# serenedb/serenedb

Measured on NVIDIA H100. Metric: filter->GROUP BY throughput (BASELINE.json configs[1]; bm25 object = configs[2]), higher is better.
Workload: dtype int64+f64

## Files before the change

### serenedb_b200/csrc/column_kernels.cuh

```cuda
#pragma once

#include "device_common.cuh"

namespace sdbg {

constexpr int kMaxPreds = 4;

struct ColDev {
  const void* values;
  const uint64_t* validity;
  int32_t type;
  int32_t pad;
};
struct PredDev {
  ColDev col;
  int32_t op;
  int32_t pad;
  int64_t lo_i, hi_i;
  double lo_f, hi_f;
};
struct PredSet {
  PredDev p[kMaxPreds];
  int32_t n;
  int32_t pad;
};

__device__ __forceinline__ bool col_valid(const ColDev& c, uint64_t r) {
  return c.validity == nullptr || ((__ldg(c.validity + (r >> 6)) >> (r & 63)) & 1ull);
}
__device__ __forceinline__ bool cmp_i64(int op, long long v, long long lo, long long hi) {
  switch (op) {
    case 0: return v < lo; case 1: return v <= lo; case 2: return v > lo; case 3: return v >= lo;
    case 4: return v == lo; case 5: return v != lo; default: return v >= lo && v <= hi;
  }
}
__device__ __forceinline__ bool cmp_f64(int op, double v, double lo, double hi) {
  switch (op) {
    case 0: return v < lo; case 1: return v <= lo; case 2: return v > lo; case 3: return v >= lo;
    case 4: return v == lo; case 5: return v != lo; default: return v >= lo && v <= hi;
  }
}

__device__ __forceinline__ uint32_t pred2(const PredDev& p, uint64_t r, uint64_t rows) {
  uint32_t valid = 3u;
  if (p.col.validity) valid = (col_valid(p.col, r) ? 1u : 0u) | ((r + 1 < rows && col_valid(p.col, r + 1)) ? 2u : 0u);
  if (p.op == 7) return (~valid) & 3u;
  if (p.op == 8) return valid;
  uint32_t m = 0;
  if (p.col.type == 2) {
    const int2 v = *reinterpret_cast<const int2*>(static_cast<const int*>(p.col.values) + r);
    m = (cmp_i64(p.op, v.x, p.lo_i, p.hi_i) ? 1u : 0u) | (cmp_i64(p.op, v.y, p.lo_i, p.hi_i) ? 2u : 0u);
  } else {
    const uint4 raw = ld_stream_v4(static_cast<const char*>(p.col.values) + r * 8);
    if (p.col.type == 1) {
      const double a = __longlong_as_double((static_cast<long long>(raw.y) << 32) | raw.x);
      const double b = __longlong_as_double((static_cast<long long>(raw.w) << 32) | raw.z);
      m = (cmp_f64(p.op, a, p.lo_f, p.hi_f) ? 1u : 0u) | (cmp_f64(p.op, b, p.lo_f, p.hi_f) ? 2u : 0u);
    } else {
      const long long a = (static_cast<long long>(raw.y) << 32) | raw.x;
      const long long b = (static_cast<long long>(raw.w) << 32) | raw.z;
      m = (cmp_i64(p.op, a, p.lo_i, p.hi_i) ? 1u : 0u) | (cmp_i64(p.op, b, p.lo_i, p.hi_i) ? 2u : 0u);
    }
  }
  return m & valid;
}

__device__ __forceinline__ uint32_t preds2(const PredSet& ps, uint64_t r, uint64_t rows) {
  uint32_t m = (r + 1 < rows) ? 3u : 1u;
#pragma unroll
  for (int i = 0; i < kMaxPreds; ++i) {
    if (i < ps.n) m &= pred2(ps.p[i], r, rows);
  }
  return m;
}

__device__ __forceinline__ bool pred1(const PredDev& p, uint64_t r) {
  const bool valid = col_valid(p.col, r);
  if (p.op >= 7) return (p.op == 8) == valid;
  if (!valid) return false;
  bool in;
  if (p.col.type == 1) {
    const double v = __ldg(static_cast<const double*>(p.col.values) + r);
    in = v >= p.lo_f && v <= p.hi_f;
  } else {
    const long long v = p.col.type == 2 ? static_cast<long long>(__ldg(static_cast<const int*>(p.col.values) + r))
                                        : __ldg(static_cast<const long long*>(p.col.values) + r);
    in = v >= p.lo_i && v <= p.hi_i;
  }
  return in != (p.op == 5);
}

__device__ __forceinline__ bool preds_row(const PredSet& ps, uint64_t r) {
  if (ps.n == 0) return true;
  if (!pred1(ps.p[0], r)) return false;
#pragma unroll 1
  for (int i = 1; i < ps.n; ++i)
    if (!pred1(ps.p[i], r)) return false;
  return true;
}

__device__ __forceinline__ void load2_i64(const ColDev& c, uint64_t r, long long& a, long long& b) {
  if (c.type == 2) {
    const int2 v = *reinterpret_cast<const int2*>(static_cast<const int*>(c.values) + r);
    a = v.x; b = v.y;
  } else {
    const uint4 raw = ld_stream_v4(static_cast<const char*>(c.values) + r * 8);
    a = (static_cast<long long>(raw.y) << 32) | raw.x;
    b = (static_cast<long long>(raw.w) << 32) | raw.z;
  }
}
__device__ __forceinline__ void load2_f64(const ColDev& c, uint64_t r, double& a, double& b) {
  const uint4 raw = ld_stream_v4(static_cast<const char*>(c.values) + r * 8);
  a = __longlong_as_double((static_cast<long long>(raw.y) << 32) | raw.x);
  b = __longlong_as_double((static_cast<long long>(raw.w) << 32) | raw.z);
}

__global__ void __launch_bounds__(256)
filter_bitmap_kernel(const PredSet ps, uint64_t rows, unsigned long long* __restrict__ mask_out) {
  const uint64_t words = (rows + 63) / 64;
  const uint32_t lane = threadIdx.x & 31u;
  for (uint64_t w = (uint64_t(blockIdx.x) * blockDim.x + threadIdx.x) >> 5; w < words;
       w += (uint64_t(gridDim.x) * blockDim.x) >> 5) {
    const uint64_t r = w * 64 + 2ull * lane;
    const uint32_t m = r < rows ? preds2(ps, r, rows) : 0u;
    const uint32_t b0 = __ballot_sync(kFull, m & 1u);
    const uint32_t b1 = __ballot_sync(kFull, m & 2u);
    if (lane == 0) {
      unsigned long long x = 0;
      for (int l = 0; l < 32; ++l) {
        x |= static_cast<unsigned long long>((b0 >> l) & 1u) << (2 * l);
        x |= static_cast<unsigned long long>((b1 >> l) & 1u) << (2 * l + 1);
      }
      mask_out[w] = x;
    }
  }
}

struct CountSumOut {
  unsigned long long count;
  unsigned long long sum_lo;
  long long sum_hi;
  double sum_f;
};

__device__ __forceinline__ void add128(unsigned long long& lo, long long& hi, long long v) {
  const unsigned long long nlo = lo + static_cast<unsigned long long>(v);
  hi += (v < 0 ? -1ll : 0ll) + (nlo < lo ? 1ll : 0ll);
  lo = nlo;
}
__device__ __forceinline__ void add128u(unsigned long long& lo, long long& hi, unsigned long long alo, long long ahi) {
  const unsigned long long nlo = lo + alo;
  hi += ahi + (nlo < lo ? 1ll : 0ll);
  lo = nlo;
}

__global__ void __launch_bounds__(256)
filter_count_sum_kernel(const PredSet ps, const ColDev sum_col, int has_sum, uint64_t rows,
                        CountSumOut* __restrict__ partials, unsigned int* __restrict__ done_counter, CountSumOut* host_out,
                        unsigned long long* host_seq, unsigned long long seq) {
  unsigned long long cnt = 0, lo = 0;
  long long hi = 0;
  double sf = 0.0;
  const uint64_t stride = uint64_t(gridDim.x) * blockDim.x * 2ull;
  for (uint64_t r = (uint64_t(blockIdx.x) * blockDim.x + threadIdx.x) * 2ull; r < rows; r += stride) {
    const uint32_t m = preds2(ps, r, rows);
    if (has_sum) {
      uint32_t mv = m;
      if (sum_col.validity) mv &= (col_valid(sum_col, r) ? 1u : 0u) | ((r + 1 < rows && col_valid(sum_col, r + 1)) ? 2u : 0u);
      if (sum_col.type == 1) {
        double a, b; load2_f64(sum_col, r, a, b);
        if (mv & 1u) sf += a;
        if (mv & 2u) sf += b;
      } else {
        long long a, b; load2_i64(sum_col, r, a, b);
        if (mv & 1u) add128(lo, hi, a);
        if (mv & 2u) add128(lo, hi, b);
      }
    }
    cnt += __popc(m);
  }
#pragma unroll
  for (int o = 16; o > 0; o >>= 1) {
    cnt += __shfl_xor_sync(kFull, cnt, o);
    const unsigned long long olo = __shfl_xor_sync(kFull, lo, o);
    const long long ohi = __shfl_xor_sync(kFull, hi, o);
    add128u(lo, hi, olo, ohi);
    sf += __shfl_xor_sync(kFull, sf, o);
  }
  __shared__ CountSumOut s[8];
  __shared__ bool s_last;
  const uint32_t lane = threadIdx.x & 31u, warp = threadIdx.x >> 5;
  if (lane == 0) { s[warp].count = cnt; s[warp].sum_lo = lo; s[warp].sum_hi = hi; s[warp].sum_f = sf; }
  __syncthreads();
  if (threadIdx.x == 0) {
    CountSumOut t = s[0];
    for (uint32_t w = 1; w < blockDim.x / 32u; ++w) {
      t.count += s[w].count; add128u(t.sum_lo, t.sum_hi, s[w].sum_lo, s[w].sum_hi); t.sum_f += s[w].sum_f;
    }
    partials[blockIdx.x] = t;
    __threadfence();
    s_last = atomicAdd(done_counter, 1u) == gridDim.x - 1u;
  }
  __syncthreads();
  if (s_last) {
    __threadfence();
    CountSumOut t = {0, 0, 0, 0.0};
    for (uint32_t b = threadIdx.x; b < gridDim.x; b += blockDim.x) {
      const volatile CountSumOut* p = partials + b;
      t.count += p->count; add128u(t.sum_lo, t.sum_hi, p->sum_lo, p->sum_hi); t.sum_f += p->sum_f;
    }
#pragma unroll
    for (int o = 16; o > 0; o >>= 1) {
      t.count += __shfl_xor_sync(kFull, t.count, o);
      const unsigned long long olo = __shfl_xor_sync(kFull, t.sum_lo, o);
      const long long ohi = __shfl_xor_sync(kFull, t.sum_hi, o);
      add128u(t.sum_lo, t.sum_hi, olo, ohi);
      t.sum_f += __shfl_xor_sync(kFull, t.sum_f, o);
    }
    __syncthreads();
    if (lane == 0) s[warp] = t;
    __syncthreads();
    if (threadIdx.x == 0) {
      CountSumOut r = s[0];
      for (uint32_t w = 1; w < blockDim.x / 32u; ++w) {
        r.count += s[w].count; add128u(r.sum_lo, r.sum_hi, s[w].sum_lo, s[w].sum_hi); r.sum_f += s[w].sum_f;
      }
      partials[gridDim.x] = r;
      if (host_out != nullptr) {
        *host_out = r;
        __threadfence_system();
        if (host_seq != nullptr) *reinterpret_cast<volatile unsigned long long*>(host_seq) = seq;
      }
      *done_counter = 0u;
    }
  }
}

struct GroupSlot {
  unsigned long long count;
  long long sum_lo;
  long long sum_hi;
  double sum_f;
};
static_assert(sizeof(GroupSlot) == 32, "one L2 sector per group");

struct GroupByParams {
  PredSet ps;
  ColDev key, sum_i, sum_f;
  int32_t has_sum_i, has_sum_f;
  int32_t wide_int;
  int32_t count_f;
  int64_t key_min;
  uint64_t key_span;
  uint64_t rows;
  GroupSlot* table;
  unsigned long long* cnt_f;
  unsigned long long* out_of_range;
};

__device__ __forceinline__ void group_update(const GroupByParams& P, long long key, long long v, bool v_ok,
                                             double w, bool w_ok) {
  const unsigned long long idx = static_cast<unsigned long long>(key - P.key_min);
  if (idx >= P.key_span) { atomicAdd(P.out_of_range, 1ull); return; }
  GroupSlot* g = P.table + idx;
  atomicAdd(&g->count, 1ull);
  if (P.has_sum_i && v_ok) {
    if (P.wide_int) {
      atomicAdd(reinterpret_cast<unsigned long long*>(&g->sum_lo), static_cast<unsigned long long>(v) & 0xFFFFFFFFull);
      atomicAdd(reinterpret_cast<unsigned long long*>(&g->sum_hi), static_cast<unsigned long long>(v >> 32));
    } else {
      atomicAdd(reinterpret_cast<unsigned long long*>(&g->sum_lo), static_cast<unsigned long long>(v));
    }
  }
  if (P.has_sum_f && w_ok) {
    atomicAdd(&g->sum_f, w);
    if (P.count_f) atomicAdd(P.cnt_f + idx, 1ull);
  }
}

template <int kUnroll>
__global__ void __launch_bounds__(256)
filter_groupby_kernel(const GroupByParams P) {
  const uint64_t tile = uint64_t(blockDim.x) * 2ull * kUnroll;
  for (uint64_t base = uint64_t(blockIdx.x) * tile; base < P.rows; base += uint64_t(gridDim.x) * tile) {
    uint32_t m[kUnroll];
    long long k0[kUnroll], k1[kUnroll], v0[kUnroll], v1[kUnroll];
    double w0[kUnroll], w1[kUnroll];
#pragma unroll
    for (int u = 0; u < kUnroll; ++u) {
      const uint64_t r = base + (uint64_t(u) * blockDim.x + threadIdx.x) * 2ull;
      m[u] = 0; k0[u] = k1[u] = v0[u] = v1[u] = 0; w0[u] = w1[u] = 0.0;
      if (r < P.rows) {
        m[u] = preds2(P.ps, r, P.rows);
        load2_i64(P.key, r, k0[u], k1[u]);
        if (P.has_sum_i) load2_i64(P.sum_i, r, v0[u], v1[u]);
        if (P.has_sum_f) load2_f64(P.sum_f, r, w0[u], w1[u]);
      }
    }
#pragma unroll
    for (int u = 0; u < kUnroll; ++u) {
      if (!m[u]) continue;
      const uint64_t r = base + (uint64_t(u) * blockDim.x + threadIdx.x) * 2ull;
      bool vi0 = true, vi1 = true, wf0 = true, wf1 = true;
      if (P.has_sum_i && P.sum_i.validity) { vi0 = col_valid(P.sum_i, r); vi1 = r + 1 < P.rows && col_valid(P.sum_i, r + 1); }
      if (P.has_sum_f && P.sum_f.validity) { wf0 = col_valid(P.sum_f, r); wf1 = r + 1 < P.rows && col_valid(P.sum_f, r + 1); }
      if (m[u] & 1u) group_update(P, k0[u], v0[u], vi0, w0[u], wf0);
      if (m[u] & 2u) group_update(P, k1[u], v1[u], vi1, w1[u], wf1);
    }
  }
}

constexpr int kMaxStreams = 7;

struct ForBlockDev { long long base; uint32_t bits; uint32_t off8; };
constexpr uint32_t kForGroupRows = 2048;
constexpr int kTypeFor = 3;

struct TmaGroupByParams {
  const void* src[kMaxStreams];
  int32_t elem[kMaxStreams];
  uint32_t off[kMaxStreams + 1];
  int32_t n_streams;
  int32_t n_preds;
  uint32_t pred_off[kMaxPreds];
  int32_t pred_type[kMaxPreds];
  int32_t pred_negate[kMaxPreds];
  int64_t pred_lo[kMaxPreds];
  uint64_t pred_span[kMaxPreds];
  uint32_t key_off, sum_i_off, sum_f_off;
  int32_t key_type, sum_i_type;
  int32_t has_sum_i, has_sum_f;
  int32_t wide_int;
  int32_t debug_skip;
  int32_t pack_shift, pack_tables;
  int64_t pack_bias;
  int64_t key_min;
  uint64_t key_span;
  uint64_t rows;
  GroupSlot* table;
  unsigned long long* out_of_range;
  const uint8_t* skip;
  const ForBlockDev* hdr[kMaxStreams];
  int32_t pred_stream[kMaxPreds];
  int32_t key_stream, sum_i_stream;
};
constexpr uint32_t kZoneRows = 2048;

__host__ __device__ __forceinline__ long long fkey(long long bits) { return bits ^ ((bits >> 63) & 0x7FFFFFFFFFFFFFFFll); }

__device__ __forceinline__ void fix_limbs(double w, int limb, int eunit, long long& l0, long long& l1) {
  const long long bits = __double_as_longlong(w);
  const int ex = int((bits >> 52) & 0x7FF);
  unsigned long long mant = static_cast<unsigned long long>(bits) & 0xFFFFFFFFFFFFFull;
  if (ex) mant |= 1ull << 52;
  const int s = (ex ? ex : 1) - 1075 - eunit;
  unsigned long long lo, hi = 0ull;
  if (s >= 0) { lo = mant << s; if (s) hi = mant >> (64 - s); }
  else lo = s > -64 ? mant >> (-s) : 0ull;
  l0 = static_cast<long long>(lo & ((1ull << limb) - 1ull));
  l1 = static_cast<long long>((lo >> limb) | (hi << (64 - limb)));
  if (bits < 0) { l0 = -l0; l1 = -l1; }
}
__host__ __device__ __forceinline__ double fix_total(long long s0, long long s1, int limb, int eunit) {
  long long hi = s1 >> (64 - limb);
  unsigned long long lo = static_cast<unsigned long long>(s1) << limb;
  const unsigned long long lo2 = lo + static_cast<unsigned long long>(s0);
  hi += (s0 >> 63) + (lo2 < lo ? 1 : 0);
  lo = lo2;
  const bool neg = hi < 0;
  if (neg) { lo = ~lo + 1ull; hi = ~hi + (lo == 0ull ? 1 : 0); }
  const double mag = static_cast<double>(static_cast<unsigned long long>(hi)) * 18446744073709551616.0 + static_cast<double>(lo);
  return scalbn(neg ? -mag : mag, eunit);
}

template <int kType>
__device__ __forceinline__ void load2(const unsigned char* col, uint32_t r, long long (&v)[2]) {
  if (kType == 2) {
    const int2 x = *reinterpret_cast<const int2*>(col + size_t(r) * 4u);
    v[0] = x.x; v[1] = x.y;
  } else {
    const longlong2 x = *reinterpret_cast<const longlong2*>(col + size_t(r) * 8u);
    v[0] = x.x; v[1] = x.y;
  }
}
template <int kType>
__device__ __forceinline__ uint32_t range2(const unsigned char* col, uint32_t r, long long lo, unsigned long long span) {
  long long v[2];
  load2<kType>(col, r, v);
  if (kType == 1) { v[0] = fkey(v[0]); v[1] = fkey(v[1]); }
  return (static_cast<unsigned long long>(v[0] - lo) <= span ? 1u : 0u) | (static_cast<unsigned long long>(v[1] - lo) <= span ? 2u : 0u);
}
__device__ __forceinline__ void unpack2(const unsigned char* col, uint32_t r, const uint4 h, long long (&v)[2]) {
  const unsigned long long* w = reinterpret_cast<const unsigned long long*>(col);
  const uint32_t bits = h.z;
  const long long base = static_cast<long long>((static_cast<unsigned long long>(h.y) << 32) | h.x);
  const unsigned long long mask = bits >= 64u ? ~0ull : (1ull << bits) - 1ull;
#pragma unroll
  for (int j = 0; j < 2; ++j) {
    const uint32_t bit = (r + uint32_t(j)) * bits, wi = bit >> 6, sh = bit & 63u;
    unsigned long long x = w[wi] >> sh;
    if (sh + bits > 64u) x |= w[wi + 1] << (64u - sh);
    v[j] = base + static_cast<long long>(x & mask);
  }
}
__device__ __forceinline__ uint32_t range2_for(const unsigned char* col, uint32_t r, const uint4 h, long long lo, unsigned long long span) {
  long long v[2];
  unpack2(col, r, h, v);
  return (static_cast<unsigned long long>(v[0] - lo) <= span ? 1u : 0u) | (static_cast<unsigned long long>(v[1] - lo) <= span ? 2u : 0u);
}

constexpr int kGroupByStages = 3;
constexpr int kGroupByTileRows = 512;
constexpr int kGroupByConsumerWarps = 8;
template <bool kPacked, bool kFor>
__global__ void __launch_bounds__((kGroupByConsumerWarps + 1) * 32)
filter_groupby_tma_kernel(const TmaGroupByParams P) {
  constexpr int kStages = kGroupByStages, kTileRows = kGroupByTileRows, kConsumerWarps = kGroupByConsumerWarps;
  extern __shared__ __align__(128) unsigned char smem[];
  __shared__ __align__(8) uint64_t full_bar[kStages], empty_bar[kStages];
  static_assert(!kFor || (kForGroupRows % kTileRows == 0 && kTileRows % 128 == 0), "a tile's packed slice must be 16-byte aligned");

  const uint32_t tid = threadIdx.x, warp = tid >> 5, lane = tid & 31u;
  if (tid == 0) {
    for (int s = 0; s < kStages; ++s) { mbar_init(&full_bar[s], 1u); mbar_init(&empty_bar[s], kConsumerWarps); }
    asm volatile("fence.mbarrier_init.release.cluster;" ::: "memory");
  }
  __syncthreads();
  const uint32_t stage_bytes = P.off[P.n_streams];
  const uint64_t n_tiles = (P.rows + kTileRows - 1) / kTileRows;
  uint4* const pk_hdr = reinterpret_cast<uint4*>(smem + size_t(kStages) * stage_bytes);

  if (warp == kConsumerWarps) {
    if (kFor) {
      const bool mine = lane < uint32_t(P.n_streams);
      const ForBlockDev* hp = mine ? P.hdr[lane] : nullptr;
      const char* src = mine ? static_cast<const char*>(P.src[lane]) : nullptr;
      const uint32_t elem = mine ? uint32_t(P.elem[lane]) : 0u, soff = mine ? P.off[lane] : 0u;
      auto header = [&](uint64_t t) { return __ldg(reinterpret_cast<const uint4*>(hp + (t * kTileRows) / kForGroupRows)); };
      uint4 nh = make_uint4(0u, 0u, 0u, 0u);
      uint64_t nh_tile = ~0ull;
      uint32_t it = 0;
      for (uint64_t tile = blockIdx.x; tile < n_tiles; tile += gridDim.x) {
        if (P.skip != nullptr && P.skip[(tile * kTileRows) / kZoneRows]) continue;
        uint4 h = make_uint4(0u, 0u, 0u, 0u);
        if (hp != nullptr) h = nh_tile == tile ? nh : header(tile);
        const uint64_t next = tile + gridDim.x;
        if (hp != nullptr && next < n_tiles && (P.skip == nullptr || !P.skip[(next * kTileRows) / kZoneRows])) { nh = header(next); nh_tile = next; }
        const uint32_t st = it % kStages, use = it / kStages;
        ++it;
        const uint64_t row0 = tile * kTileRows;
        const uint32_t nrows = uint32_t(min(static_cast<unsigned long long>(kTileRows), static_cast<unsigned long long>(P.rows - row0)));
        uint32_t bytes = 0u;
        const char* g = nullptr;
        if (hp != nullptr) {
          bytes = (nrows * h.z + 127u) / 128u * 16u;
          g = src + uint64_t(h.w) * 8u + (row0 % kForGroupRows) * h.z / 8u;
        } else if (mine) {
          bytes = (nrows * elem + 15u) & ~15u;
          g = src + row0 * elem;
        }
        const uint32_t total = __reduce_add_sync(kFull, bytes);
        if (lane == 0) mbar_wait(&empty_bar[st], (use & 1u) ^ 1u);
        for (int s = 0; s < P.n_streams; ++s) {
          uint4 x;
          x.x = __shfl_sync(kFull, h.x, s); x.y = __shfl_sync(kFull, h.y, s); x.z = __shfl_sync(kFull, h.z, s); x.w = __shfl_sync(kFull, h.w, s);
          if (lane == 0) pk_hdr[st * kMaxStreams + s] = x;
        }
        if (lane == 0) mbar_arrive_expect_tx(&full_bar[st], total);
        __syncwarp();
        if (bytes != 0u) bulk_g2s(smem + size_t(st) * stage_bytes + soff, g, bytes, &full_bar[st]);
      }
      return;
    }
    if (lane == 0) {
      uint32_t it = 0;
      for (uint64_t tile = blockIdx.x; tile < n_tiles; tile += gridDim.x) {
        if (P.skip != nullptr && P.skip[(tile * kTileRows) / kZoneRows]) continue;
        const uint32_t st = it % kStages, use = it / kStages;
        ++it;
        mbar_wait(&empty_bar[st], (use & 1u) ^ 1u);
        const uint64_t row0 = tile * kTileRows;
        const uint32_t nrows = uint32_t(min(static_cast<unsigned long long>(kTileRows), static_cast<unsigned long long>(P.rows - row0)));
        uint32_t total = 0;
        for (int s = 0; s < P.n_streams; ++s) total += (nrows * uint32_t(P.elem[s]) + 15u) & ~15u;
        mbar_arrive_expect_tx(&full_bar[st], total);
        unsigned char* dst = smem + size_t(st) * stage_bytes;
        for (int s = 0; s < P.n_streams; ++s) {
          const uint32_t bytes = (nrows * uint32_t(P.elem[s]) + 15u) & ~15u;
          bulk_g2s(dst + P.off[s], static_cast<const char*>(P.src[s]) + row0 * uint64_t(P.elem[s]), bytes, &full_bar[st]);
        }
      }
    }
    return;
  }

  uint32_t it = 0;
  for (uint64_t tile = blockIdx.x; tile < n_tiles; tile += gridDim.x) {
    if (P.skip != nullptr && P.skip[(tile * kTileRows) / kZoneRows]) continue;
    const uint32_t st = it % kStages, use = it / kStages;
    ++it;
    mbar_wait(&full_bar[st], use & 1u);
    const unsigned char* base = smem + size_t(st) * stage_bytes;
    const uint64_t row0 = tile * kTileRows;
    const uint32_t nrows = uint32_t(min(static_cast<unsigned long long>(kTileRows), static_cast<unsigned long long>(P.rows - row0)));
    const uint32_t pack_word = kPacked ? uint32_t(tile % uint64_t(P.pack_tables)) : 0u;
    const uint4* const hst = pk_hdr + st * kMaxStreams;
    for (uint32_t rb = warp * 64u; rb < nrows; rb += kConsumerWarps * 64u) {
      const uint32_t r = rb + 2u * lane;
      uint32_t m = r + 1u < nrows ? 3u : r < nrows ? 1u : 0u;
#pragma unroll
      for (int i = 0; i < kMaxPreds; ++i) {
        if (i < P.n_preds) {
          const unsigned char* col = base + P.pred_off[i];
          uint32_t in;
          if (kFor && P.pred_type[i] == kTypeFor) in = range2_for(col, r, hst[P.pred_stream[i]], P.pred_lo[i], P.pred_span[i]);
          else switch (P.pred_type[i]) {
            case 0: in = range2<0>(col, r, P.pred_lo[i], P.pred_span[i]); break;
            case 1: in = range2<1>(col, r, P.pred_lo[i], P.pred_span[i]); break;
            default: in = range2<2>(col, r, P.pred_lo[i], P.pred_span[i]); break;
          }
          m &= P.pred_negate[i] ? ~in : in;
        }
      }
      if (m == 0u) continue;
      long long key[2], v[2] = {0, 0};
      double w[2] = {0.0, 0.0};
      if (kFor && P.key_type == kTypeFor) unpack2(base + P.key_off, r, hst[P.key_stream], key);
      else if (P.key_type == 2) load2<2>(base + P.key_off, r, key); else load2<0>(base + P.key_off, r, key);
      if (kPacked || P.has_sum_i) {
        if (kFor && P.sum_i_type == kTypeFor) unpack2(base + P.sum_i_off, r, hst[P.sum_i_stream], v);
        else if (P.sum_i_type == 2) load2<2>(base + P.sum_i_off, r, v); else load2<0>(base + P.sum_i_off, r, v);
      }
      if (P.has_sum_f) {
        const double2 x = *reinterpret_cast<const double2*>(base + P.sum_f_off + size_t(r) * 8u);
        w[0] = x.x; w[1] = x.y;
      }
#pragma unroll
      for (int j = 0; j < 2; ++j) {
        if (!(m & (1u << j))) continue;
        const unsigned long long idx = static_cast<unsigned long long>(key[j] - P.key_min);
        if (idx >= P.key_span) { atomicAdd(P.out_of_range, 1ull); continue; }
        unsigned long long* g = reinterpret_cast<unsigned long long*>(P.table + idx);
        if (kPacked) {
          if (!(P.debug_skip & 3)) atomicAdd(g + pack_word, (1ull << P.pack_shift) + static_cast<unsigned long long>(v[j] - P.pack_bias));
        } else {
          if (!(P.debug_skip & 1)) atomicAdd(g, 1ull);
          if (P.has_sum_i && !(P.debug_skip & 2)) {
            if (P.wide_int) {
              atomicAdd(g + 1, static_cast<unsigned long long>(v[j]) & 0xFFFFFFFFull);
              atomicAdd(g + 2, static_cast<unsigned long long>(v[j] >> 32));
            } else {
              atomicAdd(g + 1, static_cast<unsigned long long>(v[j]));
            }
          }
        }
        if (P.has_sum_f && !(P.debug_skip & 4)) atomicAdd(reinterpret_cast<double*>(g + 3), w[j]);
      }
    }
    __syncwarp();
    if (lane == 0) mbar_arrive(&empty_bar[st]);
  }
}

template <int kType>
__global__ void __launch_bounds__(256)
zonemap_kernel(const unsigned char* __restrict__ values, uint64_t rows, long long* __restrict__ zone ) {
  const uint32_t lane = threadIdx.x & 31u;
  const uint64_t n_blocks = (rows + kZoneRows - 1) / kZoneRows;
  for (uint64_t b = (uint64_t(blockIdx.x) * blockDim.x + threadIdx.x) >> 5; b < n_blocks; b += (uint64_t(gridDim.x) * blockDim.x) >> 5) {
    long long mn = 0x7FFFFFFFFFFFFFFFll, mx = -0x7FFFFFFFFFFFFFFFll - 1;
    const uint64_t r0 = b * kZoneRows, r1 = min(rows, r0 + kZoneRows);
    for (uint64_t r = r0 + lane; r < r1; r += 32u) {
      long long v;
      if (kType == 2) v = reinterpret_cast<const int*>(values)[r];
      else v = reinterpret_cast<const long long*>(values)[r];
      if (kType == 1) v = fkey(v);
      mn = min(mn, v); mx = max(mx, v);
    }
#pragma unroll
    for (int o = 16; o > 0; o >>= 1) { mn = min(mn, __shfl_xor_sync(kFull, mn, o)); mx = max(mx, __shfl_xor_sync(kFull, mx, o)); }
    if (lane == 0) { zone[2 * b] = mn; zone[2 * b + 1] = mx; }
  }
}

constexpr uint8_t kZoneCheck = 0, kZoneDead = 1, kZonePass = 2;

struct ZoneVerdictParams {
  const long long* zone[kMaxPreds];
  long long lo[kMaxPreds];
  unsigned long long span[kMaxPreds];
  int negate[kMaxPreds];
  int n_preds;
  int pass;
  uint64_t n_blocks;
};
__host__ __device__ __forceinline__ uint8_t zone_verdict(const ZoneVerdictParams& Z, const long long* const* zone, uint64_t b) {
  bool dead = false, all = Z.pass != 0;
  for (int i = 0; i < Z.n_preds; ++i) {
    if (zone[i] == nullptr) { all = false; continue; }
    const long long mn = zone[i][2 * b], mx = zone[i][2 * b + 1];
    const long long lo = Z.lo[i];
    const bool hi_below = static_cast<unsigned long long>(mn - lo) > Z.span[i] && mn > lo;
    const bool lo_above = mx < lo;
    const bool inside = mn >= lo && static_cast<unsigned long long>(mx - lo) <= Z.span[i];
    if (Z.negate[i]) { dead |= Z.span[i] == 0ull && mn == lo && mx == lo; all &= hi_below || lo_above; }
    else { dead |= hi_below || lo_above; all &= inside; }
  }
  return dead ? kZoneDead : all ? kZonePass : kZoneCheck;
}

__global__ void __launch_bounds__(256)
zone_verdict_kernel(const ZoneVerdictParams Z, uint8_t* __restrict__ skip, unsigned long long* __restrict__ counter) {
  unsigned long long mine = 0;
  for (uint64_t b = uint64_t(blockIdx.x) * blockDim.x + threadIdx.x; b < Z.n_blocks; b += uint64_t(gridDim.x) * blockDim.x) {
    const uint8_t v = zone_verdict(Z, Z.zone, b);
    skip[b] = v;
    mine += v == kZoneDead ? 1ull : 0ull;
  }
  if (counter == nullptr) return;
  mine = warp_sum64(mine);
  if ((threadIdx.x & 31u) == 0u && mine) atomicAdd(counter, mine);
}

struct ChainDev {
  PredSet ps;
  const uint8_t* zone;
  uint32_t n_zones;
  uint32_t pad;
};

__device__ __forceinline__ bool chain_pass(const ChainDev& f, uint32_t doc) {
  const uint64_t r = uint64_t(doc) - 1u;
  if (f.zone != nullptr) {
    const uint8_t v = __ldg(f.zone + r / kZoneRows);
    if (v != kZoneCheck) return v == kZonePass;
  }
  return preds_row(f.ps, r);
}

struct HashSlot {
  long long key;
  unsigned long long count;
  long long sum_lo, sum_hi;
  double sum_f;
  unsigned long long cnt_f;
};
constexpr long long kEmptyKey = static_cast<long long>(0x8000000000000000ull);

struct HashGroupByParams {
  PredSet ps;
  ColDev key, sum_i, sum_f;
  int32_t has_sum_i, has_sum_f;
  uint64_t rows;
  HashSlot* table;
  uint64_t capacity;
  unsigned int* overflow;
};

__device__ __forceinline__ uint64_t hash_key(long long k) {
  unsigned long long z = static_cast<unsigned long long>(k) * 0x9E3779B97F4A7C15ull;
  z ^= z >> 32;
  return z;
}

__device__ __forceinline__ void hash_update(const HashGroupByParams& P, long long key, long long v, bool v_ok, double w, bool w_ok) {
  HashSlot* g = nullptr;
  if (key == kEmptyKey) {
    g = P.table + P.capacity;
    g->key = key;
  } else {
    uint64_t h = hash_key(key) & (P.capacity - 1);
    for (uint64_t probes = 0; probes < P.capacity; ++probes) {
      long long cur = *reinterpret_cast<volatile long long*>(&P.table[h].key);
      if (cur == kEmptyKey) cur = static_cast<long long>(atomicCAS(reinterpret_cast<unsigned long long*>(&P.table[h].key),
                                                                   static_cast<unsigned long long>(kEmptyKey), static_cast<unsigned long long>(key)));
      if (cur == kEmptyKey || cur == key) { g = P.table + h; break; }
      h = (h + 1) & (P.capacity - 1);
    }
    if (!g) { atomicExch(P.overflow, 1u); return; }
  }
  atomicAdd(&g->count, 1ull);
  if (P.has_sum_i && v_ok) {
    atomicAdd(reinterpret_cast<unsigned long long*>(&g->sum_lo), static_cast<unsigned long long>(v) & 0xFFFFFFFFull);
    atomicAdd(reinterpret_cast<unsigned long long*>(&g->sum_hi), static_cast<unsigned long long>(v >> 32));
  }
  if (P.has_sum_f && w_ok) { atomicAdd(&g->sum_f, w); atomicAdd(&g->cnt_f, 1ull); }
}

__global__ void __launch_bounds__(256)
hash_init_kernel(HashSlot* table, uint64_t n) {
  for (uint64_t i = uint64_t(blockIdx.x) * blockDim.x + threadIdx.x; i < n; i += uint64_t(gridDim.x) * blockDim.x) {
    HashSlot s; s.key = kEmptyKey; s.count = 0; s.sum_lo = 0; s.sum_hi = 0; s.sum_f = 0.0; s.cnt_f = 0;
    table[i] = s;
  }
}

__global__ void __launch_bounds__(256)
filter_groupby_hash_kernel(const HashGroupByParams P) {
  const uint64_t stride = uint64_t(gridDim.x) * blockDim.x * 2ull;
  for (uint64_t r = (uint64_t(blockIdx.x) * blockDim.x + threadIdx.x) * 2ull; r < P.rows; r += stride) {
    const uint32_t m = preds2(P.ps, r, P.rows);
    if (!m) continue;
    long long k0, k1, v0 = 0, v1 = 0;
    double w0 = 0, w1 = 0;
    load2_i64(P.key, r, k0, k1);
    if (P.has_sum_i) load2_i64(P.sum_i, r, v0, v1);
    if (P.has_sum_f) load2_f64(P.sum_f, r, w0, w1);
    bool vi0 = true, vi1 = true, wf0 = true, wf1 = true;
    if (P.has_sum_i && P.sum_i.validity) { vi0 = col_valid(P.sum_i, r); vi1 = r + 1 < P.rows && col_valid(P.sum_i, r + 1); }
    if (P.has_sum_f && P.sum_f.validity) { wf0 = col_valid(P.sum_f, r); wf1 = r + 1 < P.rows && col_valid(P.sum_f, r + 1); }
    if (m & 1u) hash_update(P, k0, v0, vi0, w0, wf0);
    if (m & 2u) hash_update(P, k1, v1, vi1, w1, wf1);
  }
}

__global__ void __launch_bounds__(256)
groupby_pack_kernel(const GroupSlot* __restrict__ table, const unsigned long long* __restrict__ cnt_f,
                    uint64_t span, long long* __restrict__ d_i64, double* __restrict__ d_f64,
                    int pack_shift, int pack_tables, long long pack_bias) {
  for (uint64_t i = uint64_t(blockIdx.x) * blockDim.x + threadIdx.x; i < span; i += uint64_t(gridDim.x) * blockDim.x) {
    GroupSlot g = table[i];
    if (pack_tables) {
      const unsigned long long w[3] = {g.count, static_cast<unsigned long long>(g.sum_lo), static_cast<unsigned long long>(g.sum_hi)};
      const unsigned long long mask = (1ull << pack_shift) - 1ull;
      unsigned long long cnt = 0, sum = 0;
      for (int t = 0; t < pack_tables; ++t) { cnt += w[t] >> pack_shift; sum += w[t] & mask; }
      g.count = cnt;
      g.sum_lo = static_cast<long long>(sum + static_cast<unsigned long long>(pack_bias) * cnt);
      g.sum_hi = 0;
    }
    d_i64[i] = static_cast<long long>(g.count);
    d_i64[span + i] = g.sum_lo;
    d_i64[2 * span + i] = g.sum_hi;
    d_i64[3 * span + i] = cnt_f ? static_cast<long long>(cnt_f[i]) : static_cast<long long>(g.count);
    d_f64[i] = g.sum_f;
  }
}

__global__ void __launch_bounds__(256)
minmax_i64_kernel(const ColDev col, uint64_t rows, long long* __restrict__ out ) {
  long long mn = 0x7FFFFFFFFFFFFFFFll, mx = -0x7FFFFFFFFFFFFFFFll - 1;
  for (uint64_t r = uint64_t(blockIdx.x) * blockDim.x + threadIdx.x; r < rows; r += uint64_t(gridDim.x) * blockDim.x) {
    if (!col_valid(col, r)) continue;
    const long long v = col.type == 2 ? static_cast<long long>(static_cast<const int*>(col.values)[r])
                                      : static_cast<const long long*>(col.values)[r];
    mn = min(mn, v); mx = max(mx, v);
  }
#pragma unroll
  for (int o = 16; o > 0; o >>= 1) { mn = min(mn, __shfl_xor_sync(kFull, mn, o)); mx = max(mx, __shfl_xor_sync(kFull, mx, o)); }
  if ((threadIdx.x & 31u) == 0) { atomicMin(out, mn); atomicMax(out + 1, mx); }
}

__host__ __device__ __forceinline__ unsigned long long synth_hash(unsigned long long stream, unsigned long long index) {
  unsigned long long z = (0x5EDB2026ull ^ (stream << 48) ^ index) + 0x9E3779B97F4A7C15ull;
  z = (z ^ (z >> 30)) * 0xBF58476D1CE4E5B9ull;
  z = (z ^ (z >> 27)) * 0x94D049BB133111EBull;
  return z ^ (z >> 31);
}
__global__ void __launch_bounds__(256)
synth_column_kernel(unsigned long long stream, int kind, uint64_t row0, uint64_t rows, void* __restrict__ out) {
  for (uint64_t i = uint64_t(blockIdx.x) * blockDim.x + threadIdx.x; i < rows; i += uint64_t(gridDim.x) * blockDim.x) {
    const unsigned long long h = synth_hash(stream, row0 + i);
    switch (kind) {
      case 0: static_cast<long long*>(out)[i] = static_cast<long long>(h % 100000ull); break;
      case 1: static_cast<long long*>(out)[i] = static_cast<long long>(h % 1000000ull); break;
      case 2: static_cast<double*>(out)[i] = static_cast<double>(h >> 11) * 0x1.0p-53; break;
      case 3: static_cast<long long*>(out)[i] = static_cast<long long>(h % 2001ull) - 1000ll; break;
      case 4: static_cast<double*>(out)[i] = static_cast<double>(h >> 11) * 0x1.0p-53 * 1000.0; break;
      case 6: static_cast<int*>(out)[i] = static_cast<int>(h % 1000000ull); break;
      case 7: static_cast<long long*>(out)[i] = static_cast<long long>((row0 + i) / 100ull); break;
      default: static_cast<long long*>(out)[i] = static_cast<long long>(h); break;
    }
  }
}

template <typename T>
__global__ void __launch_bounds__(256)
gather_rows_kernel(const T* __restrict__ values, const unsigned long long* __restrict__ validity, const uint32_t* __restrict__ docs,
                   uint64_t n, uint64_t rows, T* __restrict__ out, unsigned char* __restrict__ out_valid) {
  for (uint64_t i = uint64_t(blockIdx.x) * blockDim.x + threadIdx.x; i < n; i += uint64_t(gridDim.x) * blockDim.x) {
    const uint64_t r = uint64_t(docs[i]) - 1ull;
    const bool inside = r < rows;
    const bool ok = inside && (validity == nullptr || ((validity[r >> 6] >> (r & 63ull)) & 1ull));
    out[i] = ok ? values[r] : T(0);
    if (out_valid != nullptr) out_valid[i] = ok ? 1u : 0u;
  }
}

__device__ __forceinline__ long long for_value(const ForBlockDev& h, const unsigned long long* w, uint32_t i) {
  unsigned long long v = 0ull;
  if (h.bits != 0u) {
    const unsigned long long mask = h.bits >= 64u ? ~0ull : ((1ull << h.bits) - 1ull);
    const uint64_t bit = uint64_t(i) * h.bits;
    const uint32_t sh = uint32_t(bit & 63ull);
    const unsigned long long lo = w[bit >> 6] >> sh;
    const unsigned long long hi = (sh != 0u && sh + h.bits > 64u) ? (w[(bit >> 6) + 1ull] << (64u - sh)) : 0ull;
    v = (lo | hi) & mask;
  }
  return h.base + static_cast<long long>(v);
}

__global__ void __launch_bounds__(256)
for_unpack_kernel(const ForBlockDev* __restrict__ headers, const unsigned long long* __restrict__ words, uint64_t rows,
                  long long* __restrict__ out) {
  const uint64_t n_groups = (rows + kForGroupRows - 1) / kForGroupRows;
  const uint32_t lane = threadIdx.x & 31u;
  for (uint64_t g = (uint64_t(blockIdx.x) * blockDim.x + threadIdx.x) >> 5; g < n_groups; g += (uint64_t(gridDim.x) * blockDim.x) >> 5) {
    const ForBlockDev h = headers[g];
    const uint64_t row0 = g * kForGroupRows;
    const uint32_t n = (rows - row0 < kForGroupRows) ? uint32_t(rows - row0) : kForGroupRows;
    for (uint32_t i = lane; i < n; i += 32u) out[row0 + i] = for_value(h, words + h.off8, i);
  }
}

__global__ void __launch_bounds__(256)
for_stats_kernel(const long long* __restrict__ values, const ForBlockDev* __restrict__ packed_hdr,
                 const unsigned long long* __restrict__ words, uint64_t rows, long long* __restrict__ zone,
                 ForBlockDev* __restrict__ hdr, unsigned long long* __restrict__ n_words) {
  const uint64_t n_groups = (rows + kForGroupRows - 1) / kForGroupRows;
  const uint32_t lane = threadIdx.x & 31u;
  for (uint64_t g = (uint64_t(blockIdx.x) * blockDim.x + threadIdx.x) >> 5; g < n_groups; g += (uint64_t(gridDim.x) * blockDim.x) >> 5) {
    const uint64_t row0 = g * kForGroupRows;
    const uint32_t n = (rows - row0 < kForGroupRows) ? uint32_t(rows - row0) : kForGroupRows;
    long long mn = 0x7FFFFFFFFFFFFFFFll, mx = -0x7FFFFFFFFFFFFFFFll - 1;
    for (uint32_t i = lane; i < n; i += 32u) {
      const long long v = words ? for_value(packed_hdr[g], words + packed_hdr[g].off8, i) : values[row0 + i];
      mn = min(mn, v); mx = max(mx, v);
    }
#pragma unroll
    for (int o = 16; o > 0; o >>= 1) { mn = min(mn, __shfl_xor_sync(kFull, mn, o)); mx = max(mx, __shfl_xor_sync(kFull, mx, o)); }
    if (lane == 0) {
      zone[2 * g] = mn; zone[2 * g + 1] = mx;
      if (!words) {
        const unsigned long long span = static_cast<unsigned long long>(mx) - static_cast<unsigned long long>(mn);
        const uint32_t bits = span == 0ull ? 0u : uint32_t(64 - __clzll(static_cast<long long>(span)));
        ForBlockDev h; h.base = mn; h.bits = bits; h.off8 = 0u;
        hdr[g] = h;
        n_words[g] = (uint64_t(n) * bits + 63u) / 64u;
      }
    }
  }
}

__global__ void __launch_bounds__(256)
for_pack_kernel(const long long* __restrict__ values, const ForBlockDev* __restrict__ stats_hdr,
                const unsigned long long* __restrict__ offsets, uint64_t rows, ForBlockDev* __restrict__ hdr,
                unsigned long long* __restrict__ words) {
  const uint64_t n_groups = (rows + kForGroupRows - 1) / kForGroupRows;
  const uint32_t lane = threadIdx.x & 31u;
  for (uint64_t g = (uint64_t(blockIdx.x) * blockDim.x + threadIdx.x) >> 5; g < n_groups; g += (uint64_t(gridDim.x) * blockDim.x) >> 5) {
    ForBlockDev h = stats_hdr[g];
    h.off8 = uint32_t(offsets[g]);
    const uint64_t row0 = g * kForGroupRows;
    const uint32_t n = (rows - row0 < kForGroupRows) ? uint32_t(rows - row0) : kForGroupRows;
    if (lane == 0) hdr[g] = h;
    const uint32_t nw = uint32_t(offsets[g + 1] - offsets[g]);
    for (uint32_t wi = lane; wi < nw; wi += 32u) {
      const uint64_t b0 = uint64_t(wi) * 64u;
      const uint32_t i0 = uint32_t(b0 / h.bits), i1 = min(n - 1u, uint32_t((b0 + 63u) / h.bits));
      unsigned long long word = 0ull;
      for (uint32_t i = i0; i <= i1; ++i) {
        const unsigned long long d = static_cast<unsigned long long>(values[row0 + i]) - static_cast<unsigned long long>(h.base);
        const uint64_t p = uint64_t(i) * h.bits;
        word |= p >= b0 ? d << (p - b0) : d >> (b0 - p);
      }
      words[h.off8 + wi] = word;
    }
    if (g + 1 == n_groups && lane == 0) words[offsets[n_groups]] = 0ull;
  }
}

}
```

### serenedb_b200/csrc/device_common.cuh

```cuda
#pragma once

#include <cuda_runtime.h>
#include <stdint.h>

namespace sdbg {

constexpr uint32_t kWarp = 32;
constexpr unsigned kFull = 0xFFFFFFFFu;

__device__ __forceinline__ uint4 ld_stream_v4(const void* p) {
  uint4 r;
  asm volatile("ld.global.nc.L1::no_allocate.v4.u32 {%0,%1,%2,%3}, [%4];"
               : "=r"(r.x), "=r"(r.y), "=r"(r.z), "=r"(r.w) : "l"(p));
  return r;
}
__device__ __forceinline__ uint4 ld_ro_v4(const uint4* p) { return __ldg(p); }

__device__ __forceinline__ uint32_t warp_incl_scan(uint32_t v, uint32_t lane) {
#pragma unroll
  for (int o = 1; o < 32; o <<= 1) {
    const uint32_t t = __shfl_up_sync(kFull, v, o);
    if (lane >= uint32_t(o)) v += t;
  }
  return v;
}
__device__ __forceinline__ uint32_t warp_sum(uint32_t v) {
#pragma unroll
  for (int o = 16; o > 0; o >>= 1) v += __shfl_xor_sync(kFull, v, o);
  return v;
}
__device__ __forceinline__ unsigned long long warp_sum64(unsigned long long v) {
#pragma unroll
  for (int o = 16; o > 0; o >>= 1) v += __shfl_xor_sync(kFull, v, o);
  return v;
}
__device__ __forceinline__ double warp_sum_f64(double v) {
#pragma unroll
  for (int o = 16; o > 0; o >>= 1) v += __shfl_xor_sync(kFull, v, o);
  return v;
}

__device__ __forceinline__ uint32_t smem_u32(const void* p) { return static_cast<uint32_t>(__cvta_generic_to_shared(p)); }
__device__ __forceinline__ void mbar_init(uint64_t* bar, uint32_t count) {
  asm volatile("mbarrier.init.shared::cta.b64 [%0], %1;" :: "r"(smem_u32(bar)), "r"(count) : "memory");
}
__device__ __forceinline__ void mbar_arrive_expect_tx(uint64_t* bar, uint32_t bytes) {
  asm volatile("mbarrier.arrive.expect_tx.shared::cta.b64 _, [%0], %1;" :: "r"(smem_u32(bar)), "r"(bytes) : "memory");
}
__device__ __forceinline__ void mbar_arrive(uint64_t* bar) {
  asm volatile("mbarrier.arrive.shared::cta.b64 _, [%0];" :: "r"(smem_u32(bar)) : "memory");
}
__device__ __forceinline__ void mbar_wait(uint64_t* bar, uint32_t parity) {
  const uint32_t addr = smem_u32(bar);
  uint32_t ok;
  do {
    asm volatile("{\n\t.reg .pred p;\n\tmbarrier.try_wait.parity.shared::cta.b64 p, [%1], %2;\n\tselp.u32 %0, 1, 0, p;\n\t}"
                 : "=r"(ok) : "r"(addr), "r"(parity) : "memory");
  } while (!ok);
}
__device__ __forceinline__ void bulk_g2s(void* dst_smem, const void* src_gmem, uint32_t bytes, uint64_t* bar) {
  asm volatile("cp.async.bulk.shared::cluster.global.mbarrier::complete_tx::bytes [%0], [%1], %2, [%3];"
               :: "r"(smem_u32(dst_smem)), "l"(src_gmem), "r"(bytes), "r"(smem_u32(bar)) : "memory");
}

__device__ __host__ __forceinline__ unsigned long long make_key(float score, uint32_t ordinal) {
#ifdef __CUDA_ARCH__
  const uint32_t bits = __float_as_uint(score);
#else
  uint32_t bits; memcpy(&bits, &score, 4);
#endif
  return (static_cast<unsigned long long>(bits) << 32) | static_cast<unsigned long long>(~ordinal);
}

__device__ __forceinline__ void block_sort_desc(unsigned long long* s, uint32_t n) {
  for (uint32_t k = 2; k <= n; k <<= 1) {
    for (uint32_t j = k >> 1; j > 0; j >>= 1) {
      for (uint32_t i = threadIdx.x; i < n; i += blockDim.x) {
        const uint32_t p = i ^ j;
        if (p > i) {
          const unsigned long long a = s[i], b = s[p];
          const bool desc = (i & k) == 0;
          if ((a < b) == desc) { s[i] = b; s[p] = a; }
        }
      }
      __syncthreads();
    }
  }
}


__device__ __forceinline__ unsigned long long block_select_topk(unsigned long long* keys, uint32_t n_slots, uint32_t k,
                                                                uint32_t* hist) {
  const uint32_t tid = threadIdx.x, lane = tid & 31u, warp = tid >> 5, nwarps = blockDim.x >> 5;
  unsigned long long prefix = 0ull, mask = 0ull;
  uint32_t need = k;
  for (int shift = 56; shift >= 0; shift -= 8) {
    if (tid < 256) hist[tid] = 0u;
    __syncthreads();
    for (uint32_t i = tid; i < n_slots; i += blockDim.x) {
      const unsigned long long v = keys[i];
      if (v != 0ull && (v & mask) == prefix) atomicAdd(&hist[(v >> shift) & 255ull], 1u);
    }
    __syncthreads();
    if (warp == 0) {
      uint32_t c[8], sum = 0;
#pragma unroll
      for (int j = 0; j < 8; ++j) { c[j] = hist[255 - 8 * int(lane) - j]; sum += c[j]; }
      uint32_t run = warp_incl_scan(sum, lane) - sum;
      uint32_t found = 0xFFFFFFFFu, need_in = 0;
#pragma unroll
      for (int j = 0; j < 8; ++j) {
        if (found == 0xFFFFFFFFu && run < need && run + c[j] >= need) { found = 255u - 8u * lane - uint32_t(j); need_in = need - run; }
        run += c[j];
      }
      const uint32_t who = __ballot_sync(kFull, found != 0xFFFFFFFFu);
      if (who == 0u) { if (lane == 0) { hist[256] = 0xFFFFFFFFu; hist[257] = 0u; } }
      else if (lane == uint32_t(__ffs(who) - 1)) { hist[256] = found; hist[257] = need_in; }
    }
    __syncthreads();
    const uint32_t digit = hist[256];
    need = hist[257];
    __syncthreads();
    if (digit == 0xFFFFFFFFu) return 0ull;
    prefix |= static_cast<unsigned long long>(digit) << shift;
    mask |= 0xFFull << shift;
  }
  const unsigned long long kth = prefix;
  uint32_t written = 0;
  for (uint32_t t0 = 0; t0 < n_slots; t0 += blockDim.x * 4u) {
    unsigned long long v[4];
    uint32_t keep = 0;
#pragma unroll
    for (uint32_t i = 0; i < 4; ++i) {
      const uint32_t idx = t0 + tid * 4u + i;
      v[i] = idx < n_slots ? keys[idx] : 0ull;
      keep += (v[i] != 0ull && v[i] >= kth) ? 1u : 0u;
    }
    const uint32_t incl = warp_incl_scan(keep, lane);
    if (lane == 31) hist[warp] = incl;
    __syncthreads();
    uint32_t base = written + incl - keep, total = 0;
    for (uint32_t w = 0; w < nwarps; ++w) { if (w < warp) base += hist[w]; total += hist[w]; }
#pragma unroll
    for (uint32_t i = 0; i < 4; ++i) if (v[i] != 0ull && v[i] >= kth) keys[base++] = v[i];
    written += total;
    __syncthreads();
  }
  for (uint32_t i = written + tid; i < n_slots; i += blockDim.x) keys[i] = 0ull;
  __syncthreads();
  return kth;
}

}
```

Baseline: 79200.

## Add L2 eviction hints and release pipeline stage before group-by atomics

Streaming column TMA loads now carry an L2 evict_first policy, and the group-by table reductions use red.global with an evict_last policy so the hash/direct table stays resident in L2. Consumer warps now process exactly one 64-row strip per tile and arrive on the empty barrier right after reading shared memory, before issuing the global atomics. This lets the producer refill the stage while the reductions are still in flight. It also adds a static_assert that ties the tile size to the consumer warp count.

```diff
diff --git a/serenedb_b200/csrc/column_kernels.cuh b/serenedb_b200/csrc/column_kernels.cuh
--- a/serenedb_b200/csrc/column_kernels.cuh
+++ b/serenedb_b200/csrc/column_kernels.cuh
@@ -431,6 +431,7 @@
   uint4* const pk_hdr = reinterpret_cast<uint4*>(smem + size_t(kStages) * stage_bytes);
 
   if (warp == kConsumerWarps) {
+    const uint64_t stream_policy = l2_policy_evict_first();
     if (kFor) {
       const bool mine = lane < uint32_t(P.n_streams);
       const ForBlockDev* hp = mine ? P.hdr[lane] : nullptr;
@@ -468,7 +469,7 @@
         }
         if (lane == 0) mbar_arrive_expect_tx(&full_bar[st], total);
         __syncwarp();
-        if (bytes != 0u) bulk_g2s(smem + size_t(st) * stage_bytes + soff, g, bytes, &full_bar[st]);
+        if (bytes != 0u) bulk_g2s_hint(smem + size_t(st) * stage_bytes + soff, g, bytes, &full_bar[st], stream_policy);
       }
       return;
     }
@@ -487,13 +488,15 @@
         unsigned char* dst = smem + size_t(st) * stage_bytes;
         for (int s = 0; s < P.n_streams; ++s) {
           const uint32_t bytes = (nrows * uint32_t(P.elem[s]) + 15u) & ~15u;
-          bulk_g2s(dst + P.off[s], static_cast<const char*>(P.src[s]) + row0 * uint64_t(P.elem[s]), bytes, &full_bar[st]);
+          bulk_g2s_hint(dst + P.off[s], static_cast<const char*>(P.src[s]) + row0 * uint64_t(P.elem[s]), bytes, &full_bar[st], stream_policy);
         }
       }
     }
     return;
   }
 
+  static_assert(kTileRows == kConsumerWarps * 64, "each consumer warp reads exactly one 64-row strip of a tile");
+  const uint64_t table_policy = l2_policy_evict_last();
   uint32_t it = 0;
   for (uint64_t tile = blockIdx.x; tile < n_tiles; tile += gridDim.x) {
     if (P.skip != nullptr && P.skip[(tile * kTileRows) / kZoneRows]) continue;
@@ -505,26 +508,25 @@
     const uint32_t nrows = uint32_t(min(static_cast<unsigned long long>(kTileRows), static_cast<unsigned long long>(P.rows - row0)));
     const uint32_t pack_word = kPacked ? uint32_t(tile % uint64_t(P.pack_tables)) : 0u;
     const uint4* const hst = pk_hdr + st * kMaxStreams;
-    for (uint32_t rb = warp * 64u; rb < nrows; rb += kConsumerWarps * 64u) {
-      const uint32_t r = rb + 2u * lane;
-      uint32_t m = r + 1u < nrows ? 3u : r < nrows ? 1u : 0u;
-#pragma unroll
-      for (int i = 0; i < kMaxPreds; ++i) {
-        if (i < P.n_preds) {
-          const unsigned char* col = base + P.pred_off[i];
-          uint32_t in;
-          if (kFor && P.pred_type[i] == kTypeFor) in = range2_for(col, r, hst[P.pred_stream[i]], P.pred_lo[i], P.pred_span[i]);
-          else switch (P.pred_type[i]) {
-            case 0: in = range2<0>(col, r, P.pred_lo[i], P.pred_span[i]); break;
-            case 1: in = range2<1>(col, r, P.pred_lo[i], P.pred_span[i]); break;
-            default: in = range2<2>(col, r, P.pred_lo[i], P.pred_span[i]); break;
-          }
-          m &= P.pred_negate[i] ? ~in : in;
+    const uint32_t r = warp * 64u + 2u * lane;
+    uint32_t m = r + 1u < nrows ? 3u : r < nrows ? 1u : 0u;
+#pragma unroll
+    for (int i = 0; i < kMaxPreds; ++i) {
+      if (i < P.n_preds) {
+        const unsigned char* col = base + P.pred_off[i];
+        uint32_t in;
+        if (kFor && P.pred_type[i] == kTypeFor) in = range2_for(col, r, hst[P.pred_stream[i]], P.pred_lo[i], P.pred_span[i]);
+        else switch (P.pred_type[i]) {
+          case 0: in = range2<0>(col, r, P.pred_lo[i], P.pred_span[i]); break;
+          case 1: in = range2<1>(col, r, P.pred_lo[i], P.pred_span[i]); break;
+          default: in = range2<2>(col, r, P.pred_lo[i], P.pred_span[i]); break;
         }
-      }
-      if (m == 0u) continue;
-      long long key[2], v[2] = {0, 0};
-      double w[2] = {0.0, 0.0};
+        m &= P.pred_negate[i] ? ~in : in;
+      }
+    }
+    long long key[2] = {0, 0}, v[2] = {0, 0};
+    double w[2] = {0.0, 0.0};
+    if (m != 0u) {
       if (kFor && P.key_type == kTypeFor) unpack2(base + P.key_off, r, hst[P.key_stream], key);
       else if (P.key_type == 2) load2<2>(base + P.key_off, r, key); else load2<0>(base + P.key_off, r, key);
       if (kPacked || P.has_sum_i) {
@@ -535,30 +537,30 @@
         const double2 x = *reinterpret_cast<const double2*>(base + P.sum_f_off + size_t(r) * 8u);
         w[0] = x.x; w[1] = x.y;
       }
-#pragma unroll
-      for (int j = 0; j < 2; ++j) {
-        if (!(m & (1u << j))) continue;
-        const unsigned long long idx = static_cast<unsigned long long>(key[j] - P.key_min);
-        if (idx >= P.key_span) { atomicAdd(P.out_of_range, 1ull); continue; }
-        unsigned long long* g = reinterpret_cast<unsigned long long*>(P.table + idx);
-        if (kPacked) {
-          if (!(P.debug_skip & 3)) atomicAdd(g + pack_word, (1ull << P.pack_shift) + static_cast<unsigned long long>(v[j] - P.pack_bias));
-        } else {
-          if (!(P.debug_skip & 1)) atomicAdd(g, 1ull);
-          if (P.has_sum_i && !(P.debug_skip & 2)) {
-            if (P.wide_int) {
-              atomicAdd(g + 1, static_cast<unsigned long long>(v[j]) & 0xFFFFFFFFull);
-              atomicAdd(g + 2, static_cast<unsigned long long>(v[j] >> 32));
-            } else {
-              atomicAdd(g + 1, static_cast<unsigned long long>(v[j]));
-            }
+    }
+    __syncwarp();
+    if (lane == 0) mbar_arrive(&empty_bar[st]);
+#pragma unroll
+    for (int j = 0; j < 2; ++j) {
+      if (!(m & (1u << j))) continue;
+      const unsigned long long idx = static_cast<unsigned long long>(key[j] - P.key_min);
+      if (idx >= P.key_span) { atomicAdd(P.out_of_range, 1ull); continue; }
+      unsigned long long* g = reinterpret_cast<unsigned long long*>(P.table + idx);
+      if (kPacked) {
+        if (!(P.debug_skip & 3)) red_add_hint(g + pack_word, (1ull << P.pack_shift) + static_cast<unsigned long long>(v[j] - P.pack_bias), table_policy);
+      } else {
+        if (!(P.debug_skip & 1)) red_add_hint(g, 1ull, table_policy);
+        if (P.has_sum_i && !(P.debug_skip & 2)) {
+          if (P.wide_int) {
+            red_add_hint(g + 1, static_cast<unsigned long long>(v[j]) & 0xFFFFFFFFull, table_policy);
+            red_add_hint(g + 2, static_cast<unsigned long long>(v[j] >> 32), table_policy);
+          } else {
+            red_add_hint(g + 1, static_cast<unsigned long long>(v[j]), table_policy);
           }
         }
-        if (P.has_sum_f && !(P.debug_skip & 4)) atomicAdd(reinterpret_cast<double*>(g + 3), w[j]);
-      }
-    }
-    __syncwarp();
-    if (lane == 0) mbar_arrive(&empty_bar[st]);
+      }
+      if (P.has_sum_f && !(P.debug_skip & 4)) red_add_hint(reinterpret_cast<double*>(g + 3), w[j], table_policy);
+    }
   }
 }
 
diff --git a/serenedb_b200/csrc/device_common.cuh b/serenedb_b200/csrc/device_common.cuh
--- a/serenedb_b200/csrc/device_common.cuh
+++ b/serenedb_b200/csrc/device_common.cuh
@@ -61,6 +61,27 @@
 __device__ __forceinline__ void bulk_g2s(void* dst_smem, const void* src_gmem, uint32_t bytes, uint64_t* bar) {
   asm volatile("cp.async.bulk.shared::cluster.global.mbarrier::complete_tx::bytes [%0], [%1], %2, [%3];"
                :: "r"(smem_u32(dst_smem)), "l"(src_gmem), "r"(bytes), "r"(smem_u32(bar)) : "memory");
+}
+__device__ __forceinline__ void bulk_g2s_hint(void* dst_smem, const void* src_gmem, uint32_t bytes, uint64_t* bar, uint64_t policy) {
+  asm volatile("cp.async.bulk.shared::cluster.global.mbarrier::complete_tx::bytes.L2::cache_hint [%0], [%1], %2, [%3], %4;"
+               :: "r"(smem_u32(dst_smem)), "l"(src_gmem), "r"(bytes), "r"(smem_u32(bar)), "l"(policy) : "memory");
+}
+
+__device__ __forceinline__ uint64_t l2_policy_evict_first() {
+  uint64_t p;
+  asm volatile("createpolicy.fractional.L2::evict_first.b64 %0, 1.0;" : "=l"(p));
+  return p;
+}
+__device__ __forceinline__ uint64_t l2_policy_evict_last() {
+  uint64_t p;
+  asm volatile("createpolicy.fractional.L2::evict_last.b64 %0, 1.0;" : "=l"(p));
+  return p;
+}
+__device__ __forceinline__ void red_add_hint(unsigned long long* p, unsigned long long v, uint64_t policy) {
+  asm volatile("red.global.add.L2::cache_hint.u64 [%0], %1, %2;" :: "l"(__cvta_generic_to_global(p)), "l"(v), "l"(policy) : "memory");
+}
+__device__ __forceinline__ void red_add_hint(double* p, double v, uint64_t policy) {
+  asm volatile("red.global.add.L2::cache_hint.f64 [%0], %1, %2;" :: "l"(__cvta_generic_to_global(p)), "d"(v), "l"(policy) : "memory");
 }
 
 __device__ __host__ __forceinline__ unsigned long long make_key(float score, uint32_t ordinal) {
```

Result: no change. 79440, median of 6 (+0.3%).
